# bitlayer-org/tap-stark

Measured on AMD Instinct MI355X. Metric: trace cells/sec (proofs/sec alongside), 2^20x64 BabyBear trace, higher is better.
Workload: dtype u32

## Files before the change

tap-stark_amd/csrc/abi.cpp:

```cpp
#include <stdio.h>
#include <string.h>

#include <algorithm>
#include <atomic>
#include <chrono>
#include <mutex>
#include <thread>
#include <memory>
#include <string>
#include <vector>

#include "abi_types.hpp"
#include "blake3.hpp"
#include "collect.hpp"
#include "derive.hpp"
#include "jit.hpp"
#include "join.hpp"
#include "logup.hpp"
#include "prover_internal.hpp"
#include "scan.hpp"
#include "sort.hpp"

static const ts::AirProgram& ready_prog(const ts_air* air) { return const_cast<ts_air*>(air)->a.ready(); }

// ... 438 lines not shown
    memcpy(buf, s.c_str(), s.size() + 1);
    return TS_OK;
}

ts_status ts_ctx_set_replay(ts_ctx* ctx, int mode) {
    if (!ctx || mode < 0 || mode > 2) return TS_ERR_INVALID;
    return guard(ctx, [&] {
        ctx->ctx.sync();
        if (mode == 1) ctx->ctx.replay_log.clear();
        ctx->ctx.replay_pos = 0;
        ctx->ctx.replay_mode = mode;
    });
}
ts_status ts_ctx_set_kernel_timing(ts_ctx* ctx, int enabled) {
    if (!ctx) return TS_ERR_INVALID;
    return guard(ctx, [&] {
        ctx->ctx.take_kernel_timings();
        ctx->ctx.kernel_timing = enabled != 0;
    });
}
ts_status ts_ctx_take_kernel_timings(ts_ctx* ctx, char* buf, size_t cap) {
    if (!ctx || !buf || cap == 0) return TS_ERR_INVALID;
    return guard(ctx, [&] {
        std::string s;
        for (auto& kv : ctx->ctx.take_kernel_timings()) {
            char tmp[200];
            snprintf(tmp, sizeof tmp, "%s=%llu:%.6f;", kv.first.c_str(),
                     (unsigned long long)kv.second.first, kv.second.second);
            s += tmp;
        }
        TS_REQUIRE(s.size() + 1 <= cap, ts::TS_ERR_BUFFER, "timing buffer too small");
        memcpy(buf, s.c_str(), s.size() + 1);
    });
}

ts_status ts_ctx_graph_stats(ts_ctx* ctx, uint64_t out[4]) {
    if (!ctx || !out) return TS_ERR_INVALID;
    out[0] = out[1] = out[2] = 0;
    out[3] = ctx->ctx.bytes_reserved;
    return TS_OK;
}

ts_status ts_ctx_stat(ts_ctx* ctx, int which, uint64_t* out) {
    if (!ctx || !out) return TS_ERR_INVALID;
    switch (which) {
    case 0: case 1: case 2: case 4: *out = 0; break;
    case 3: *out = ctx->ctx.bytes_reserved; break;
    case 5: *out = ctx->ctx.local_quotient_fallbacks; break;
    case 6: *out = ctx->ctx.pow_hints_accepted; break;
    case 7: *out = ctx->ctx.pow_hints_rejected; break;
    case 8: *out = ctx->ctx.pow_host_grinds; break;
    case 9: *out = ctx->ctx.poison_fills; break;
    case 11: *out = ctx->ctx.live_blocks.size(); break;
    default: return TS_ERR_INVALID;
    }
    return TS_OK;
}

ts_status ts_bench_alu(ts_ctx* ctx, int kind, double* units_per_second) {
    if (!ctx || !units_per_second) return TS_ERR_INVALID;
    return guard(ctx, [&] { *units_per_second = ts::alu_ceiling(ctx->ctx, kind); });
}

ts_status ts_bench_stage(ts_ctx* ctx, int stage, unsigned log_n, uint32_t width, unsigned log_blowup,
                         uint32_t reps, double* ms_per_rep) {
    if (!ctx || !ms_per_rep) return TS_ERR_INVALID;
    return guard(ctx, [&] { *ms_per_rep = ts::bench_stage(ctx->ctx, stage, log_n, width, log_blowup, reps); });
}

ts_status ts_host_alloc(size_t bytes, void** out) {
    if (!out || bytes == 0) return TS_ERR_INVALID;
    *out = nullptr;
    return hipHostMalloc(out, bytes, hipHostMallocDefault) == hipSuccess ? TS_OK : TS_ERR_OOM;
}
void ts_host_free(void* p) {
    if (p) (void)hipHostFree(p);
}

static ts_matrix* new_matrix(ts::DeviceMatrix m) {
    auto h = std::make_unique<ts_matrix>();
    h->m = std::move(m);
    return h.release();
}
static ts_status matrix_from(ts_ctx* ctx, const uint32_t* src, uint64_t height, uint32_t width,
                             hipMemcpyKind kind, ts_matrix** out, bool sync = true) {
    if (!ctx || !out) return TS_ERR_INVALID;
    *out = nullptr;
    return guard(ctx, [&] {
        TS_REQUIRE(src && height >= 1 && width >= 1, ts::TS_ERR_INVALID, "matrix: empty");
        TS_REQUIRE((height & (height - 1)) == 0, ts::TS_ERR_INVALID, "matrix: height must be a power of two");
        TS_REQUIRE(height <= (1ull << 27), ts::TS_ERR_INVALID, "matrix: height > 2^27");
        auto m = std::make_unique<ts_matrix>();
        m->m.buf = ts::DevBuf<uint32_t>(&ctx->ctx, (size_t)height * width);
        m->m.height = height;
        m->m.width = width;
        m->m.layout = ts::DeviceMatrix::ROW_MAJOR;
        TS_HIP(hipMemcpyAsync(m->m.buf.p, src, (size_t)height * width * 4, kind, ctx->ctx.stream));
        if (sync) ctx->ctx.sync();
        *out = m.release();
    });
}
ts_status ts_matrix_upload(ts_ctx* ctx, const uint32_t* host, uint64_t height, uint32_t width,
                           ts_matrix** out) {
    return matrix_from(ctx, host, height, width, hipMemcpyHostToDevice, out);
}
ts_status ts_matrix_upload_async(ts_ctx* ctx, const uint32_t* host_pinned, uint64_t height,
// ... 2012 lines not shown
```

tap-stark_amd/csrc/context.cpp:

```cpp
#include <errno.h>
#include <stdio.h>
#include <time.h>
#include <stdlib.h>
#include "context.hpp"

#include <string.h>

#include "kernels.hpp"

namespace ts {

static bool poison_knob(uint32_t* word) {
    const char* e = getenv("TS_POOL_POISON");
    if (!e || !*e) return false;
    char* end = nullptr;
    errno = 0;
    const unsigned long v = strtoul(e, &end, 0);
    TS_REQUIRE(errno == 0 && end != e && *end == 0 && e[0] != '-' && v <= 0xFFFFFFFFul, TS_ERR_INVALID,
               "TS_POOL_POISON is not a 32-bit word (decimal, 0x hex or 0 octal)");
    *word = (uint32_t)v;
    return true;
}

Context::Context(int dev) : device(dev) {
    pool_debug = getenv("TS_POOL_DEBUG") != nullptr;
    poison_on = poison_knob(&poison_word);
    int count = 0;
    hipError_t e = hipGetDeviceCount(&count);
    if (e != hipSuccess || count == 0)
        throw Error(TS_ERR_HIP, "no HIP device available: the tap-stark HIP path has no CPU fallback");
    TS_REQUIRE(dev >= 0 && dev < count, TS_ERR_INVALID, "device index out of range");
    TS_HIP(hipSetDevice(dev));
    hipDeviceProp_t prop;
    TS_HIP(hipGetDeviceProperties(&prop, dev));
    num_cus = prop.multiProcessorCount;
    max_lds_per_block = prop.sharedMemPerBlock;
    arch_name = prop.gcnArchName;
    arch_name = arch_name.substr(0, arch_name.find(':'));
    TS_HIP(hipStreamCreateWithFlags(&stream, hipStreamNonBlocking));
}

Context::~Context() {
    (void)hipSetDevice(device);
    if (stream) (void)hipStreamSynchronize(stream);
    if (d_twiddle_fwd) (void)hipFree(d_twiddle_fwd);
    if (d_twiddle_inv) (void)hipFree(d_twiddle_inv);
    if (d_plant_fwd) (void)hipFree(d_plant_fwd);
    if (d_plant_inv) (void)hipFree(d_plant_inv);
    for (auto& t : scale_tables) (void)hipFree(t.d);
    for (auto& t : sel_tables)
        if (t.d) (void)hipFree(t.d);
    if (d_ticket) (void)hipFree(d_ticket);
    for (auto& kv : free_blocks) (void)hipFree(kv.second);
    for (auto& kv : live_blocks) (void)hipFree(kv.first);
    if (h_pinned) (void)hipHostFree(h_pinned);
    if (h_mailbox) (void)hipHostFree(h_mailbox);
    if (h_mailbox_big) (void)hipHostFree(h_mailbox_big);
    if (h_arena) (void)hipHostFree(h_arena);
    if (stream) (void)hipStreamDestroy(stream);
}

static size_t round_block(size_t bytes) {
    if (bytes < 512) return 512;
    if (bytes < (1u << 20)) {
        size_t r = 512;
        while (r < bytes) r <<= 1;
        return r;
    }
    const size_t g = 1u << 20;
    return (bytes + g - 1) / g * g;
}

void* Context::alloc(size_t bytes) {
    const size_t sz = round_block(bytes);
    auto it = free_blocks.find(sz);
    void* p = nullptr;
    if (it != free_blocks.end()) {
        p = it->second;
        free_blocks.erase(it);
    } else {
        TS_HIP(hipSetDevice(device));
        if (pool_debug) {
            struct timespec ts_;
            clock_gettime(CLOCK_MONOTONIC, &ts_);
            fprintf(stderr, "[ts pool %p t=%.3f ms] hipMalloc %zu KiB (reserved %zu MiB)\n", (void*)this,
                    ts_.tv_sec * 1e3 + ts_.tv_nsec * 1e-6, sz >> 10, bytes_reserved >> 20);
        }
        hipError_t e = hipMalloc(&p, sz);
        if (e != hipSuccess) {
            release_cache();
            e = hipMalloc(&p, sz);
        }
        if (e != hipSuccess) {
            (void)hipGetLastError();
            throw Error(TS_ERR_OOM, "device allocation failed");
        }
        bytes_reserved += sz;
    }
    live_blocks[p] = sz;
    if (poison_on) poison(p, sz);
    return p;
}

void Context::poison(void* p, size_t bytes) {
// ... 6 lines not shown
void Context::free(void* p) {
    if (!p) return;
    auto it = live_blocks.find(p);
    if (it == live_blocks.end()) return;
    free_blocks.emplace(it->second, p);
    live_blocks.erase(it);
}

void Context::release_cache() {
    if (stream) (void)hipStreamSynchronize(stream);
    for (auto& kv : free_blocks) {
        (void)hipFree(kv.second);
        bytes_reserved -= kv.first;
    }
    free_blocks.clear();
}

uint32_t* Context::ticket() {
    if (!d_ticket) {
        TS_HIP(hipMalloc((void**)&d_ticket, 64 * 17));
        TS_HIP(hipMemsetAsync(d_ticket, 0, 64 * 17, stream));
    }
    return d_ticket;
}

const void* Context::stage(const void* src, size_t bytes) {
    const size_t need = (bytes + 63) & ~(size_t)63;
    if (need > h_arena_bytes / 2) {
        sync();
        if (h_arena) (void)hipHostFree(h_arena);
        h_arena = nullptr;
        size_t sz = 1 << 20;
        while (sz / 2 < need) sz <<= 1;
        TS_HIP(hipHostMalloc((void**)&h_arena, sz, hipHostMallocDefault));
        h_arena_bytes = sz;
        h_arena_off = 0;
    }
    if (h_arena_off + need > h_arena_bytes) {
        sync();
        h_arena_off = 0;
    }
    void* p = h_arena + h_arena_off;
    memcpy(p, src, bytes);
    h_arena_off += need;
    return p;
}

void Context::sync_point(void* host, size_t bytes) {
    if (replay_mode == 2 && replay_pos < replay_log.size() && replay_log[replay_pos].size() == bytes) {
        memcpy(host, replay_log[replay_pos++].data(), bytes);
        return;
    }
    sync();
    if (replay_mode == 1) replay_log.emplace_back((const char*)host, (const char*)host + bytes);
}
void Context::d2h_point(void* host_dst, const void* dev_src, size_t bytes) {
    if (replay_mode == 2 && replay_pos < replay_log.size() && replay_log[replay_pos].size() == bytes) {
        memcpy(host_dst, replay_log[replay_pos++].data(), bytes);
        return;
    }
    if (bytes) TS_HIP(hipMemcpyAsync(host_dst, dev_src, bytes, hipMemcpyDeviceToHost, stream));
    sync();
    if (replay_mode == 1) replay_log.emplace_back((const char*)host_dst, (const char*)host_dst + bytes);
}

uint32_t* Context::mailbox(size_t words) {
    constexpr size_t WORDS = 16384;
    if (words > WORDS / 4) {
        if (words > h_mailbox_big_words) {
            sync();
            if (h_mailbox_big) (void)hipHostFree(h_mailbox_big);
            h_mailbox_big = nullptr;
            h_mailbox_big_words = 0;
            TS_HIP(hipHostMalloc((void**)&h_mailbox_big, words * 4, hipHostMallocDefault));
            h_mailbox_big_words = words;
        }
        return h_mailbox_big;
    }
    if (!h_mailbox) TS_HIP(hipHostMalloc((void**)&h_mailbox, WORDS * 4, hipHostMallocDefault));
    const size_t need = (words + 15) & ~(size_t)15;
    if (mailbox_off + need > WORDS) mailbox_off = 0;
    uint32_t* p = h_mailbox + mailbox_off;
    mailbox_off += need;
    return p;
}

void* Context::pinned(size_t bytes) {
    if (bytes > h_pinned_bytes) {
        if (h_pinned) {
            sync();
            (void)hipHostFree(h_pinned);
        }
        size_t sz = 1 << 16;
        while (sz < bytes) sz <<= 1;
        TS_HIP(hipHostMalloc(&h_pinned, sz, hipHostMallocDefault));
        h_pinned_bytes = sz;
    }
    return h_pinned;
}

std::map<std::string, std::pair<uint64_t, double>> Context::take_kernel_timings() {
    std::map<std::string, std::pair<uint64_t, double>> out;
    sync();
    for (auto& ev : kernel_events) {
        float ms = 0;
        (void)hipEventElapsedTime(&ms, ev.e0, ev.e1);
        auto& slot = out[ev.name];
        slot.first += 1;
        slot.second += ms;
        (void)hipEventDestroy(ev.e0);
        (void)hipEventDestroy(ev.e1);
    }
    kernel_events.clear();
    return out;
}

void Context::ensure_twiddles(unsigned log_size) {
    if (log_size <= twiddle_log && d_twiddle_fwd) return;
    TS_REQUIRE(log_size <= 27, TS_ERR_INVALID, "two-adicity of BabyBear is 27");
    sync();
    if (d_twiddle_fwd) (void)hipFree(d_twiddle_fwd);
    if (d_twiddle_inv) (void)hipFree(d_twiddle_inv);
    d_twiddle_fwd = d_twiddle_inv = nullptr;
    const size_t n = (size_t)1 << log_size;
    TS_HIP(hipMalloc((void**)&d_twiddle_fwd, n * 4));
    TS_HIP(hipMalloc((void**)&d_twiddle_inv, n * 4));
    if (poison_on) {
        poison(d_twiddle_fwd, n * 4);
        poison(d_twiddle_inv, n * 4);
    }
    twiddle_log = log_size;
    launch_build_twiddles(*this, d_twiddle_fwd, d_twiddle_inv, log_size);
}

void Context::ensure_plant_twiddles(unsigned log_size) {
    if (log_size <= plant_log && d_plant_fwd) return;
    TS_REQUIRE(log_size <= 27, TS_ERR_INVALID, "two-adicity of BabyBear is 27");
    sync();
    if (d_plant_fwd) (void)hipFree(d_plant_fwd);
    if (d_plant_inv) (void)hipFree(d_plant_inv);
    d_plant_fwd = d_plant_inv = nullptr;
    const size_t n = (size_t)1 << log_size;
    TS_HIP(hipMalloc((void**)&d_plant_fwd, n * 8));
    TS_HIP(hipMalloc((void**)&d_plant_inv, n * 8));
    if (poison_on) {
        poison(d_plant_fwd, n * 8);
        poison(d_plant_inv, n * 8);
    }
    plant_log = log_size;
    launch_build_plant_twiddles(*this, d_plant_fwd, d_plant_inv, log_size);
}

}
```

tap-stark_amd/csrc/context.hpp:

```cpp
#pragma once
#include <hip/hip_runtime.h>
#include <stdint.h>

#include <map>
#include <stdexcept>
#include <string>
#include <vector>

#include "bb.hpp"

namespace ts {

struct Error : std::runtime_error {
    int code;
    Error(int c, const std::string& m) : std::runtime_error(m), code(c) {}
};

struct FinalPolyNotConstant : Error {
    explicit FinalPolyNotConstant(const std::string& m) : Error(5 , m) {}
};

enum : int {
    TS_OK = 0,
    TS_ERR_INVALID = 1,
    TS_ERR_HIP = 2,
    TS_ERR_OOM = 3,
    TS_ERR_UNSUPPORTED = 4,
    TS_ERR_INVARIANT = 5,
    TS_ERR_BUFFER = 6,
    TS_ERR_COMM = 7,
};

#define TS_HIP(expr)                                                                        \
    do {                                                                                    \
        hipError_t _e = (expr);                                                             \
        if (_e != hipSuccess)                                                               \
            throw ts::Error(ts::TS_ERR_HIP, std::string(#expr) + ": " + hipGetErrorString(_e)); \
    } while (0)

#define TS_REQUIRE(cond, code, msg)                   \
    do {                                              \
        if (!(cond)) throw ts::Error((code), (msg));  \
    } while (0)

struct Context {
    int device = 0;
    hipStream_t stream = nullptr;
    std::string last_error;
    int num_cus = 256;
    size_t max_lds_per_block = 64 * 1024;
    std::string arch_name;

    std::multimap<size_t, void*> free_blocks;
    std::map<void*, size_t> live_blocks;
    size_t bytes_reserved = 0;
    bool pool_debug = false;
    bool poison_on = false;
    uint32_t poison_word = 0;
    uint64_t poison_fills = 0;
    void poison(void* p, size_t bytes);

    uint32_t* d_twiddle_fwd = nullptr;
    uint32_t* d_twiddle_inv = nullptr;
    unsigned twiddle_log = 0;
    uint2* d_plant_fwd = nullptr;
    uint2* d_plant_inv = nullptr;
    unsigned plant_log = 0;

    struct ScaleTable {
        unsigned log_n, log_blowup;
        uint32_t shift;
        uint32_t* d;
        size_t words;
        uint64_t last_use;
    };
    std::vector<ScaleTable> scale_tables;
    uint64_t scale_clock = 0;
    struct SelTable {
        uint32_t* d = nullptr;
        unsigned log_n = ~0u, log_qd = ~0u;
        uint32_t shift = 0;
        uint64_t last_use = 0;
    };
    SelTable sel_tables[2];
    uint64_t sel_clock = 0;

    uint32_t* d_ticket = nullptr;
    uint32_t* ticket();

    unsigned lde_pass_mask = 7;

    uint32_t* h_mailbox = nullptr;
    size_t mailbox_off = 0;
    uint32_t* h_mailbox_big = nullptr;
    size_t h_mailbox_big_words = 0;
    uint32_t* mailbox(size_t words);

    void* h_pinned = nullptr;
    size_t h_pinned_bytes = 0;
    char* h_arena = nullptr;
    size_t h_arena_bytes = 0, h_arena_off = 0;
    const void* stage(const void* src, size_t bytes);

    bool timing = false;
    std::vector<std::pair<std::string, float>> stage_ms;

    struct KernelEvent {
        const char* name;
        hipEvent_t e0, e1;
    };
    bool kernel_timing = false;
    std::vector<KernelEvent> kernel_events;
    std::map<std::string, std::pair<uint64_t, double>> take_kernel_timings();

    uint64_t pow_hints_accepted = 0, pow_hints_rejected = 0, pow_host_grinds = 0;
    uint64_t local_quotient_fallbacks = 0;

    explicit Context(int dev);
    ~Context();
    Context(const Context&) = delete;

    void* alloc(size_t bytes);
    void free(void* p);
    template <class T>
    T* alloc_n(size_t n) { return static_cast<T*>(alloc(n * sizeof(T))); }
    void release_cache();

    int replay_mode = 0;
    size_t replay_pos = 0;
    std::vector<std::vector<char>> replay_log;
    void sync_point(void* host, size_t bytes);
    void d2h_point(void* host_dst, const void* dev_src, size_t bytes);
    void* pinned(size_t bytes);
    void ensure_twiddles(unsigned log_size);
    void ensure_plant_twiddles(unsigned log_size);
    void sync() { TS_HIP(hipStreamSynchronize(stream)); }
};

// ... 77 lines not shown
```

tap-stark_amd/csrc/ntt.hip:

```cpp
#include "kernels.hpp"

namespace ts {

constexpr int SHIFT_LO_BITS = 10;

__device__ __forceinline__ uint32_t twiddle_mont(uint32_t idx) {
    if (idx == 0) return R_MOD_P;
    unsigned logm = 31 - __clz(idx);
    uint32_t i = idx - (1u << logm);
    uint32_t g27 = to_mont(TWO_ADIC_GEN_27);
    uint32_t g = mont_pow(g27, 1ull << (27 - (logm + 1)));
    uint32_t e = bitrev32(i, logm);
    return mont_pow(g, e);
}

__global__ void k_build_twiddles(uint32_t* __restrict__ W, uint32_t* __restrict__ Winv,
                                 unsigned log_size) {
    uint32_t idx = blockIdx.x * blockDim.x + threadIdx.x;
    if (idx >= (1u << log_size)) return;
    const uint32_t w = twiddle_mont(idx);
    W[idx] = w;
    Winv[idx] = mont_inv(w);
}

// ... 7 lines not shown
}

void launch_build_twiddles(Context& ctx, uint32_t* W, uint32_t* Winv, unsigned log_size) {
    uint32_t n = 1u << log_size;
    TS_LAUNCH(ctx, k_build_twiddles, dim3((n + 255) / 256), dim3(256), 0, W, Winv, log_size);
    TS_HIP(hipGetLastError());
}

void launch_build_plant_twiddles(Context& ctx, uint2* WP, uint2* WPinv, unsigned log_size) {
    uint32_t n = 1u << log_size;
    TS_LAUNCH(ctx, k_build_plant_twiddles, dim3((n + 255) / 256), dim3(256), 0, WP, WPinv, log_size);
    TS_HIP(hipGetLastError());
}

__global__ void k_build_shift_tables(uint32_t* __restrict__ lo, uint32_t* __restrict__ hi,
                                     uint32_t n_hi, uint32_t shift_mont, unsigned log_N,
                                     unsigned log_blowup, uint32_t scale_mont) {
    uint32_t beta = blockIdx.y;
    uint32_t j = blockIdx.x * blockDim.x + threadIdx.x;
    uint32_t n_lo = 1u << SHIFT_LO_BITS;
    if (j >= n_lo + n_hi) return;
    uint32_t g27 = to_mont(TWO_ADIC_GEN_27);
    uint32_t gN = mont_pow(g27, 1ull << (27 - log_N));
    uint32_t s = mont_mul(shift_mont, mont_pow(gN, bitrev32(beta, log_blowup)));
    if (j < n_lo) {
        lo[beta * n_lo + j] = mont_mul(mont_pow(s, j), scale_mont);
    } else {
        uint32_t jj = j - n_lo;
        hi[beta * n_hi + jj] = mont_pow(s, (uint64_t)jj << SHIFT_LO_BITS);
    }
}

void launch_build_shift_tables(Context& ctx, uint32_t* lo, uint32_t* hi, uint32_t n_hi,
                               uint32_t n_cosets, uint32_t shift_mont, unsigned log_N,
                               unsigned log_blowup, uint32_t scale_mont) {
    const uint32_t n_lo = 1u << SHIFT_LO_BITS;
    TS_LAUNCH(ctx, k_build_shift_tables, dim3((n_lo + n_hi + 255) / 256, n_cosets), dim3(256), 0, lo,
              hi, n_hi, shift_mont, log_N, log_blowup, scale_mont);
    TS_HIP(hipGetLastError());
}

__global__ void __launch_bounds__(256)
k_build_scale_table(const uint32_t* __restrict__ lo, const uint32_t* __restrict__ hi, uint32_t n_hi,
                    unsigned log_n, uint32_t* __restrict__ T) {
    const uint32_t beta = blockIdx.y;
    const uint64_t k = (uint64_t)blockIdx.x * blockDim.x + threadIdx.x;
    if (k >= (1ull << log_n)) return;
    const uint32_t n_lo = 1u << SHIFT_LO_BITS;
    T[((uint64_t)beta << log_n) + k] =
        mont_mul(lo[beta * n_lo + (k & (n_lo - 1))], hi[(uint64_t)beta * n_hi + (k >> SHIFT_LO_BITS)]);
}

const uint32_t* coset_scale_table(Context& ctx, unsigned log_n, unsigned log_blowup, uint32_t shift) {
    for (auto& t : ctx.scale_tables)
        if (t.log_n == log_n && t.log_blowup == log_blowup && t.shift == shift) {
            t.last_use = ++ctx.scale_clock;
            return t.d;
        }
    const uint32_t n_cosets = 1u << log_blowup;
    const size_t words = (size_t)n_cosets << log_n;
    size_t total = words * 4;
    for (auto& t : ctx.scale_tables) total += t.words * 4;
    while (!ctx.scale_tables.empty() && (ctx.scale_tables.size() >= 8 || total > (2ull << 30))) {
        size_t victim = 0;
        for (size_t i = 1; i < ctx.scale_tables.size(); i++)
            if (ctx.scale_tables[i].last_use < ctx.scale_tables[victim].last_use) victim = i;
        ctx.sync();
        total -= ctx.scale_tables[victim].words * 4;
        (void)hipFree(ctx.scale_tables[victim].d);
        ctx.scale_tables.erase(ctx.scale_tables.begin() + victim);
    }
    uint32_t* d = nullptr;
    TS_HIP(hipMalloc((void**)&d, words * 4));
    if (ctx.poison_on) ctx.poison(d, words * 4);
    const uint64_t n = 1ull << log_n;
    const uint32_t n_lo = 1u << SHIFT_LO_BITS;
    const uint32_t n_hi = log_n > (unsigned)SHIFT_LO_BITS ? 1u << (log_n - SHIFT_LO_BITS) : 1u;
    DevBuf<uint32_t> lo(&ctx, (size_t)n_cosets * n_lo), hi(&ctx, (size_t)n_cosets * n_hi);
    const uint32_t n_inv_mont = to_mont(inv_canon((uint32_t)(n % P)));
    launch_build_shift_tables(ctx, lo.p, hi.p, n_hi, n_cosets, to_mont(shift), log_n + log_blowup, log_blowup,
                              n_inv_mont);
    TS_LAUNCH(ctx, k_build_scale_table, dim3((unsigned)((n + 255) / 256), n_cosets), dim3(256), 0,
              (const uint32_t*)lo.p, (const uint32_t*)hi.p, n_hi, log_n, d);
    TS_HIP(hipGetLastError());
    ctx.scale_tables.push_back(Context::ScaleTable{log_n, log_blowup, shift, d, words, ++ctx.scale_clock});
    return d;
}

template <bool TO_COLUMNS, bool BITREV>
__global__ void __launch_bounds__(256)
k_transpose_tile(const uint32_t* __restrict__ src, uint32_t* __restrict__ dst, uint64_t h, unsigned log_h,
                 uint32_t w, uint64_t col_stride, uint32_t rm_width) {
    __shared__ uint32_t tile[64][65];
    const uint64_t p0 = (uint64_t)blockIdx.x * 64;
    const uint32_t c0 = blockIdx.y * 64;
    const uint32_t tx = threadIdx.x & 63, ty = threadIdx.x >> 6;
    auto row_of = [&](uint64_t p) -> uint64_t { return BITREV ? bitrev32((uint32_t)p, log_h) : p; };
    if (p0 + 64 <= h && c0 + 64 <= w) {
        const uint64_t rm = row_of(p0) * rm_width + c0 + tx;
        const uint64_t rm_step = BITREV ? (uint64_t)rm_width << (log_h - 6) : rm_width;
        const uint64_t cm = (uint64_t)(c0 + ty) * col_stride + p0 + tx;
        auto rm_at = [&](int k) {
            const uint32_t i = ty + 4 * (uint32_t)k;
            return rm + (uint64_t)(BITREV ? __brev(i) >> 26 : i) * rm_step;
        };
        auto cm_at = [&](int k) { return cm + (uint64_t)(4 * k) * col_stride; };
        uint32_t t[16];
#pragma unroll
        for (int k = 0; k < 16; k++) t[k] = src[TO_COLUMNS ? rm_at(k) : cm_at(k)];
#pragma unroll
        for (int k = 0; k < 16; k++) (TO_COLUMNS ? tile[ty + 4 * k][tx] : tile[tx][ty + 4 * k]) = t[k];
        __syncthreads();
#pragma unroll
        for (int k = 0; k < 16; k++) t[k] = TO_COLUMNS ? tile[tx][ty + 4 * k] : tile[ty + 4 * k][tx];
#pragma unroll
        for (int k = 0; k < 16; k++) dst[TO_COLUMNS ? cm_at(k) : rm_at(k)] = t[k];
        return;
    }
    auto rm_ok = [&](uint32_t j) { return p0 + j < h && c0 + tx < w; };
    auto cm_ok = [&](uint32_t j) { return c0 + j < w && p0 + tx < h; };
    auto rm_at = [&](uint32_t j) { return row_of(p0 + j) * rm_width + c0 + tx; };
    auto cm_at = [&](uint32_t j) { return (uint64_t)(c0 + j) * col_stride + p0 + tx; };
#pragma unroll
    for (int k = 0; k < 16; k++) {
        const uint32_t j = ty + 4 * (uint32_t)k;
        if (TO_COLUMNS ? rm_ok(j) : cm_ok(j)) (TO_COLUMNS ? tile[j][tx] : tile[tx][j]) = src[TO_COLUMNS ? rm_at(j) : cm_at(j)];
    }
    __syncthreads();
#pragma unroll
    for (int k = 0; k < 16; k++) {
        const uint32_t j = ty + 4 * (uint32_t)k;
        if (TO_COLUMNS ? cm_ok(j) : rm_ok(j)) dst[TO_COLUMNS ? cm_at(j) : rm_at(j)] = TO_COLUMNS ? tile[tx][j] : tile[j][tx];
    }
}

template <bool TO_COLUMNS, bool BITREV>
static void launch_transpose_tile(Context& ctx, const char* name, const uint32_t* src, uint32_t* dst, uint64_t h,
                                  unsigned log_h, uint32_t w, uint64_t col_stride, uint32_t rm_width) {
    if (w == 0 || h == 0) return;
// ... 28 lines not shown
```

tap-stark_amd/csrc/ntt_lde.hip:

```cpp
#include <stdlib.h>

#include <optional>
#include <type_traits>

#include "ntt_rounds.hpp"

namespace ts {

template <int LM, bool SKIP_R16 = false, class TW = uint32_t>
__global__ void __launch_bounds__(chunk_threads(LM))
k_intt_contig(uint32_t* __restrict__ data, uint64_t col_stride, unsigned log_n,
              const TW* __restrict__ Winv, uint32_t* __restrict__ data2, uint32_t gw) {
    __shared__ uint32_t s[padded(1 << LM)];
    const uint32_t c = blockIdx.x;
    uint32_t* col = blockIdx.y < gw ? data + (uint64_t)blockIdx.y * col_stride
                                    : data2 + (uint64_t)(blockIdx.y - gw) * col_stride;
    uint32_t* g = col + ((uint64_t)c << LM);
    chunk_load<LM>(s, g);
    chunk_rounds<LM, true, SKIP_R16>(s, log_n - LM, c, Winv);
    chunk_store<LM, false>(s, g);
}

__global__ void __launch_bounds__(256)
k_transpose_bitrev_r16(const uint32_t* __restrict__ src, uint32_t* __restrict__ dst, unsigned log_n,
// ... 330 lines not shown
        TS_LAUNCH_NAMED(ctx, "k_lde_mid<1>", TS_MID_K(1, TILE_ELEMS, LOG_M, false), grid1, b, 0, TS_MID_ARGS);
    else if (p.mid == NttMid::FIXED256 && p.LM == 13)
        TS_LAUNCH_NAMED(ctx, "(k_lde_mid<1, 8192, 512, 13>)", TS_MID_K(1, 8192, 13, false), grid1, b, 0, TS_MID_ARGS);
    else if (p.mid == NttMid::FIXED256)
        TS_LAUNCH_NAMED(ctx, "(k_lde_mid<1, 8192, 512, 14>)", TS_MID_K(1, 8192, 14, false), grid1, b, 0, TS_MID_ARGS);
    else
        TS_LAUNCH_NAMED(ctx, "k_lde_mid<0>", TS_MID_K(0, TILE_ELEMS, LOG_M, false), grid, b, 0, TS_MID_ARGS);
#undef TS_MID_ARGS
#undef TS_MID_K
}

void launch_contig_forward(Context& ctx, const NttPlan& p, uint32_t* data, uint64_t col_stride, uint32_t ncols,
                           uint32_t n_blocks, uint32_t gw, uint32_t own_a, uint32_t own_b) {
    const TwTables W = twiddles_fwd(ctx);
    with_chunk_log(p.LM, [&](auto lm) {
        constexpr int LM = decltype(lm)::value;
        using TW = typename ContigForm<LM>::Fwd;
        constexpr int CPW = LM == 14 ? 4 : 1;
        if (own_a != LDE_NO_OWN)
            TS_LAUNCH_NAMED(ctx, FWD_NAME[LM - 12], (k_lde_fwd_contig_own<LM, CPW, TW>),
                            dim3(p.chunks / CPW, ncols, n_blocks - 1), dim3(chunk_threads(LM)), 0, data, col_stride,
                            p.log_n, W, gw, own_a, own_b);
        else
            TS_LAUNCH_NAMED(ctx, FWD_NAME[LM - 12], (k_lde_fwd_contig<LM, CPW, TW>), dim3(p.chunks / CPW, ncols, n_blocks),
                            dim3(chunk_threads(LM)), 0, data, col_stride, p.log_n, W);
    });
}

int lde_own_coset_used(unsigned log_n, unsigned log_blowup, uint32_t shift) {
    if (const char* e = getenv("TS_LDE_OWN_COSET"); e && *e && atoi(e) == 0) return -1;
    if (log_blowup == 0 || log_n + log_blowup > 27 || ntt_plan(log_n).mid == NttMid::TILE16384) return -1;
    return lde_own_coset(log_n, log_blowup, shift);
}

void coset_lde(Context& ctx, uint32_t* evals, uint64_t in_col_stride, uint32_t ncols, unsigned log_n,
               unsigned log_blowup, uint32_t shift, uint32_t* out, uint64_t out_col_stride,
               uint32_t beta0, uint32_t n_beta, bool first_round_done, uint32_t* evals2, uint32_t shift2,
               uint32_t gw, bool stage_timers) {
    if (ncols == 0) return;
    TS_REQUIRE(evals2 == nullptr || (gw >= 1 && gw < ncols && shift2 != 0), TS_ERR_INVALID,
               "coset_lde: second matrix needs its first column and its shift");
    if (evals2 == nullptr) gw = 0xffffffffu;
    TS_REQUIRE(log_n + log_blowup <= 27, TS_ERR_INVALID, "coset_lde: log_n + log_blowup > 27");
    const NttPlan p = ntt_plan(log_n);
    ntt_require_shape(p, ncols, in_col_stride, out_col_stride, true);
    TS_REQUIRE(!first_round_done || p.fused_first_round, TS_ERR_INVARIANT,
               "coset_lde: no contiguous inverse pass at this size");
    ctx.ensure_twiddles(log_n == 0 ? 1 : log_n);
    ctx.ensure_plant_twiddles(log_n == 0 ? 1 : log_n);

    const uint32_t n_cosets = 1u << log_blowup;
    if (n_beta == 0) n_beta = n_cosets - beta0;
    TS_REQUIRE(beta0 < n_cosets && n_beta <= n_cosets - beta0, TS_ERR_INVALID, "coset_lde: coset range");
    const uint32_t* scale = coset_scale_table(ctx, log_n, log_blowup, shift);
    const uint32_t* scale2 = evals2 ? coset_scale_table(ctx, log_n, log_blowup, shift2) : nullptr;

    uint32_t own_a = LDE_NO_OWN, own_b = LDE_NO_OWN;
    if (beta0 == 0 && n_beta == n_cosets && !first_round_done && ctx.lde_pass_mask == 7u) {
        const int a = lde_own_coset_used(log_n, log_blowup, shift);
        const int b = evals2 ? lde_own_coset_used(log_n, log_blowup, shift2) : a;
        if (a >= 0 && b >= 0) {
            own_a = (uint32_t)a;
            own_b = (uint32_t)b;
            const uint64_t n = 1ull << log_n;
            if (p.two_pass)
                TS_LAUNCH_NAMED(ctx, "k_lde_own_copy", k_lde_own_copy<true>, dim3((unsigned)(n >> 12), ncols), dim3(256), 0,
                                (const uint32_t*)evals, in_col_stride, out, out_col_stride, log_n,
                                (const uint32_t*)evals2, gw, own_a, own_b);
            else
                TS_LAUNCH_NAMED(ctx, "k_lde_own_copy", k_lde_own_copy<false>, dim3((unsigned)((n + 255) / 256), ncols),
                                dim3(256), 0, (const uint32_t*)evals, in_col_stride, out, out_col_stride, log_n,
                                (const uint32_t*)evals2, gw, own_a, own_b);
        }
    }

    if (!p.two_pass) {
        launch_lde_mid(ctx, p, evals, in_col_stride, out, out_col_stride, ncols, beta0, n_beta, scale, evals2, scale2,
                       gw, own_a, own_b);
    } else {
        if (ctx.lde_pass_mask & 1u) {
            std::optional<StageTimer> t;
            if (stage_timers) t.emplace(&ctx, "lde: inverse NTT, contiguous stages");
            launch_contig_inverse(ctx, p, evals, in_col_stride, ncols, first_round_done, evals2, gw);
        }
        std::optional<StageTimer> t_rest;
        if (stage_timers) t_rest.emplace(&ctx, "lde: strided pass + forward NTT of the owned cosets");
        if (ctx.lde_pass_mask & 2u)
            launch_lde_mid(ctx, p, evals, in_col_stride, out, out_col_stride, ncols, beta0, n_beta, scale, evals2,
                           scale2, gw, own_a, own_b);
        if (ctx.lde_pass_mask & 4u) launch_contig_forward(ctx, p, out, out_col_stride, ncols, n_beta, gw, own_a, own_b);
    }
    TS_HIP(hipGetLastError());
}

}
```

tap-stark_amd/csrc/quotient.hip:

```cpp
#include <stdlib.h>

#include <algorithm>

#include "air.hpp"
#include "kernels.hpp"

namespace ts {

constexpr int SEL_BATCH = 8;

struct SelConsts {
    uint32_t zh_mont[MAX_QUOTIENT_CHUNKS];
};

__global__ void __launch_bounds__(256)
k_selectors(unsigned L, unsigned log_qd, const uint32_t* __restrict__ W, uint32_t gen_mont,
            uint32_t gn_inv_mont, SelConsts sc, uint32_t* __restrict__ is_first,
            uint32_t* __restrict__ is_last, uint32_t* __restrict__ is_transition) {
    const uint64_t total = 1ull << L;
    const uint64_t r0 = ((uint64_t)blockIdx.x * blockDim.x + threadIdx.x) * SEL_BATCH;
    if (r0 >= total) return;
    const unsigned log_n = L - log_qd;
    uint32_t d[2 * SEL_BATCH];
    uint32_t pre[2 * SEL_BATCH];
    uint32_t run = R_MOD_P;
    const int cnt = (total - r0) < (uint64_t)SEL_BATCH ? (int)(total - r0) : SEL_BATCH;
#pragma unroll
    for (int k = 0; k < SEL_BATCH; k++) {
        if (k < cnt) {
            uint64_t r = r0 + k;
            uint32_t w = L == 0 ? R_MOD_P : W[(total >> 1) + (r >> 1)];
            if (r & 1) w = neg(w);
            uint32_t x = mont_mul(gen_mont, w);
            d[2 * k] = sub(x, R_MOD_P);
            d[2 * k + 1] = sub(x, gn_inv_mont);
        } else {
            d[2 * k] = d[2 * k + 1] = R_MOD_P;
        }
        pre[2 * k] = run;
        run = mont_mul(run, d[2 * k]);
        pre[2 * k + 1] = run;
        run = mont_mul(run, d[2 * k + 1]);
    }
    uint32_t inv = mont_inv(run);
#pragma unroll
    for (int k = SEL_BATCH - 1; k >= 0; k--) {
        uint32_t inv_last = mont_mul(inv, pre[2 * k + 1]);
        inv = mont_mul(inv, d[2 * k + 1]);
        uint32_t inv_first = mont_mul(inv, pre[2 * k]);
        inv = mont_mul(inv, d[2 * k]);
        if (k < cnt) {
            uint64_t r = r0 + k;
            uint32_t c = bitrev32((uint32_t)(r >> log_n), log_qd);
            uint32_t zh = sc.zh_mont[c];
            is_first[r] = mont_mul(zh, inv_first);
            is_last[r] = mont_mul(zh, inv_last);
            is_transition[r] = d[2 * k + 1];
        }
    }
}

static void coset_vanishing(uint32_t shift, unsigned log_n, unsigned log_qd, uint32_t zh[MAX_QUOTIENT_CHUNKS]) {
    TS_REQUIRE((1u << log_qd) <= (unsigned)MAX_QUOTIENT_CHUNKS, TS_ERR_UNSUPPORTED, "quotient degree > 64 not supported");
    const uint32_t s_pow_n = pow_canon(shift, 1ull << log_n);
    const uint32_t gqd = two_adic_generator(log_qd);
    for (uint32_t c = 0; c < (1u << log_qd); c++) zh[c] = sub(mul(s_pow_n, pow_canon(gqd, c)), 1);
}

static void launch_selectors(Context& ctx, unsigned log_n, unsigned log_qd, uint32_t* is_first,
                             uint32_t* is_last, uint32_t* is_transition, uint32_t shift) {
    const unsigned L = log_n + log_qd;
    ctx.ensure_twiddles(L == 0 ? 1 : L);
    SelConsts sc;
    coset_vanishing(shift, log_n, log_qd, sc.zh_mont);
    for (uint32_t c = 0; c < (1u << log_qd); c++) sc.zh_mont[c] = to_mont(sc.zh_mont[c]);
    const uint32_t gn_inv = inv_canon(two_adic_generator(log_n));
    const uint64_t threads = (((uint64_t)1 << L) + SEL_BATCH - 1) / SEL_BATCH;
    TS_LAUNCH(ctx, k_selectors, dim3((unsigned)((threads + 255) / 256)), dim3(256), 0, L, log_qd, ctx.d_twiddle_fwd, to_mont(shift), to_mont(gn_inv), sc, is_first,
                       is_last, is_transition);
    TS_HIP(hipGetLastError());
}

const uint32_t* selector_table(Context& ctx, unsigned log_n, unsigned log_qd, uint32_t shift) {
    Context::SelTable* st = nullptr;
    for (auto& t : ctx.sel_tables)
        if (t.d && t.log_n == log_n && t.log_qd == log_qd && t.shift == shift) st = &t;
    if (!st) {
        st = ctx.sel_tables[0].last_use <= ctx.sel_tables[1].last_use ? &ctx.sel_tables[0] : &ctx.sel_tables[1];
        if (st->d) {
            ctx.sync();
            (void)hipFree(st->d);
            *st = Context::SelTable{};
        }
        const uint64_t qn = 1ull << (log_n + log_qd);
        TS_HIP(hipMalloc((void**)&st->d, 3 * qn * sizeof(uint32_t)));
        if (ctx.poison_on) ctx.poison(st->d, 3 * qn * sizeof(uint32_t));
        launch_selectors(ctx, log_n, log_qd, st->d, st->d + qn, st->d + 2 * qn, shift);
        st->log_n = log_n;
        st->log_qd = log_qd;
        st->shift = shift;
    }
    st->last_use = ++ctx.sel_clock;
    return st->d;
}

struct QuotConsts {
    uint32_t inv_zh_canonical[MAX_QUOTIENT_CHUNKS];
};

struct RegFilePlan {
    int nthreads;
    bool global;
    size_t lds_bytes;
    unsigned grid;
    uint32_t n_tiles;
    size_t scratch_words;
};

static uint64_t env_u64(const char* name, uint64_t dflt) {
    const char* e = getenv(name);
    return e && *e ? (uint64_t)atoi(e) : dflt;
}

static RegFilePlan plan_reg_file(Context& ctx, uint32_t n_regs, uint64_t rows) {
    RegFilePlan pl;
    pl.nthreads = 256;
    while (pl.nthreads > 64 && (size_t)n_regs * pl.nthreads * 4 > 48 * 1024) pl.nthreads >>= 1;
    pl.lds_bytes = (size_t)n_regs * pl.nthreads * 4;
    const size_t lds_max_regs = env_u64("TS_INTERP_LDS_MAX_REGS", 48);
    const unsigned waves_per_cu = (unsigned)env_u64("TS_INTERP_WAVES_PER_CU", 16);
    pl.global = n_regs > lds_max_regs || pl.lds_bytes > ctx.max_lds_per_block || getenv("TS_INTERP_GLOBAL_REGS") != nullptr;
    if (pl.global) pl.nthreads = 64;
    pl.n_tiles = (uint32_t)((rows + pl.nthreads - 1) / pl.nthreads);
    if (pl.global) {
        pl.lds_bytes = 0;
        uint64_t grid = std::min<uint64_t>(pl.n_tiles, (uint64_t)ctx.num_cus * waves_per_cu);
        const uint64_t slab_mb = env_u64("TS_INTERP_SLAB_MB", 4096);
        const uint64_t cap = (slab_mb << 18) / ((uint64_t)n_regs * 64);
        grid = std::max<uint64_t>(1, std::min(grid, cap));
        pl.grid = (unsigned)grid;
    } else {
        pl.grid = pl.n_tiles;
    }
    pl.scratch_words = pl.global ? (size_t)pl.grid * n_regs * 64 : 0;
    return pl;
}

template <int NTHREADS, bool GLOBAL_REGS>
__device__ __forceinline__ uint32_t* lane_regs(uint32_t* reg_slabs, uint32_t n_regs) {
    extern __shared__ uint32_t lds_regs[];
    return GLOBAL_REGS ? reg_slabs + (size_t)blockIdx.x * n_regs * NTHREADS + threadIdx.x : lds_regs + threadIdx.x;
}

template <int NTHREADS, class Row>
__device__ __forceinline__ void run_program(const uint32_t* code, uint32_t n_instr,
                                            const uint32_t* consts_mont, uint32_t* my, Row& row) {
// ... 329 lines not shown
```

Baseline: 26.58 billion.

## Share twiddle, scale and selector tables across contexts on the same device

Moves twiddle, plant-twiddle, coset scale and selector tables into a per-device registry shared by all contexts through reference-counted handles with LRU eviction, so several contexts or provers on one GPU reuse tables instead of each rebuilding them. The selector cache grows from 2 to 16 entries when shared. Builds now synchronize the stream, and refs to evicted tables are dropped at sync points. This adds mutex and ref-count bookkeeping and can raise device memory residency.

```diff
diff --git a/tap-stark_amd/csrc/abi.cpp b/tap-stark_amd/csrc/abi.cpp
--- a/tap-stark_amd/csrc/abi.cpp
+++ b/tap-stark_amd/csrc/abi.cpp
@@ -514,6 +514,8 @@
     case 8: *out = ctx->ctx.pow_host_grinds; break;
     case 9: *out = ctx->ctx.poison_fills; break;
     case 11: *out = ctx->ctx.live_blocks.size(); break;
+    case 12: *out = ctx->ctx.table_bytes(); break;
+    case 13: *out = ctx->ctx.tables_built; break;
     default: return TS_ERR_INVALID;
     }
     return TS_OK;
diff --git a/tap-stark_amd/csrc/context.cpp b/tap-stark_amd/csrc/context.cpp
--- a/tap-stark_amd/csrc/context.cpp
+++ b/tap-stark_amd/csrc/context.cpp
@@ -38,18 +38,16 @@
     arch_name = prop.gcnArchName;
     arch_name = arch_name.substr(0, arch_name.find(':'));
     TS_HIP(hipStreamCreateWithFlags(&stream, hipStreamNonBlocking));
+    tables = device_tables(dev, poison_on || !shared_tables_knob());
 }
 
 Context::~Context() {
     (void)hipSetDevice(device);
     if (stream) (void)hipStreamSynchronize(stream);
-    if (d_twiddle_fwd) (void)hipFree(d_twiddle_fwd);
-    if (d_twiddle_inv) (void)hipFree(d_twiddle_inv);
-    if (d_plant_fwd) (void)hipFree(d_plant_fwd);
-    if (d_plant_inv) (void)hipFree(d_plant_inv);
-    for (auto& t : scale_tables) (void)hipFree(t.d);
-    for (auto& t : sel_tables)
-        if (t.d) (void)hipFree(t.d);
+    table_refs.held.clear();
+    twiddle_ref.reset();
+    plant_ref.reset();
+    tables.reset();
     if (d_ticket) (void)hipFree(d_ticket);
     for (auto& kv : free_blocks) (void)hipFree(kv.second);
     for (auto& kv : live_blocks) (void)hipFree(kv.first);
@@ -162,6 +160,7 @@
         return;
     }
     sync();
+    table_refs.drop_evicted();
     if (replay_mode == 1) replay_log.emplace_back((const char*)host, (const char*)host + bytes);
 }
 void Context::d2h_point(void* host_dst, const void* dev_src, size_t bytes) {
@@ -171,6 +170,7 @@
     }
     if (bytes) TS_HIP(hipMemcpyAsync(host_dst, dev_src, bytes, hipMemcpyDeviceToHost, stream));
     sync();
+    table_refs.drop_evicted();
     if (replay_mode == 1) replay_log.emplace_back((const char*)host_dst, (const char*)host_dst + bytes);
 }
 
@@ -226,39 +226,41 @@
 }
 
 void Context::ensure_twiddles(unsigned log_size) {
-    if (log_size <= twiddle_log && d_twiddle_fwd) return;
+    if (d_twiddle_fwd && log_size <= twiddle_log && twiddle_log == tables->twiddle_log(TAB_TWIDDLE)) return;
     TS_REQUIRE(log_size <= 27, TS_ERR_INVALID, "two-adicity of BabyBear is 27");
-    sync();
-    if (d_twiddle_fwd) (void)hipFree(d_twiddle_fwd);
-    if (d_twiddle_inv) (void)hipFree(d_twiddle_inv);
-    d_twiddle_fwd = d_twiddle_inv = nullptr;
     const size_t n = (size_t)1 << log_size;
-    TS_HIP(hipMalloc((void**)&d_twiddle_fwd, n * 4));
-    TS_HIP(hipMalloc((void**)&d_twiddle_inv, n * 4));
-    if (poison_on) {
-        poison(d_twiddle_fwd, n * 4);
-        poison(d_twiddle_inv, n * 4);
-    }
-    twiddle_log = log_size;
-    launch_build_twiddles(*this, d_twiddle_fwd, d_twiddle_inv, log_size);
+    bool built = false;
+    twiddle_ref = tables->twiddles(TAB_TWIDDLE, log_size, n * 4, [&](void* fwd, void* inv) {
+        if (poison_on) {
+            poison(fwd, n * 4);
+            poison(inv, n * 4);
+        }
+        launch_build_twiddles(*this, (uint32_t*)fwd, (uint32_t*)inv, log_size);
+        sync();
+    }, &built);
+    tables_built += built;
+    d_twiddle_fwd = (uint32_t*)twiddle_ref->d[0];
+    d_twiddle_inv = (uint32_t*)twiddle_ref->d[1];
+    twiddle_log = twiddle_ref->key.a;
 }
 
 void Context::ensure_plant_twiddles(unsigned log_size) {
-    if (log_size <= plant_log && d_plant_fwd) return;
+    if (d_plant_fwd && log_size <= plant_log && plant_log == tables->twiddle_log(TAB_PLANT)) return;
     TS_REQUIRE(log_size <= 27, TS_ERR_INVALID, "two-adicity of BabyBear is 27");
-    sync();
-    if (d_plant_fwd) (void)hipFree(d_plant_fwd);
-    if (d_plant_inv) (void)hipFree(d_plant_inv);
-    d_plant_fwd = d_plant_inv = nullptr;
     const size_t n = (size_t)1 << log_size;
-    TS_HIP(hipMalloc((void**)&d_plant_fwd, n * 8));
-    TS_HIP(hipMalloc((void**)&d_plant_inv, n * 8));
-    if (poison_on) {
-        poison(d_plant_fwd, n * 8);
-        poison(d_plant_inv, n * 8);
-    }
-    plant_log = log_size;
-    launch_build_plant_twiddles(*this, d_plant_fwd, d_plant_inv, log_size);
-}
-
-}
+    bool built = false;
+    plant_ref = tables->twiddles(TAB_PLANT, log_size, n * 8, [&](void* fwd, void* inv) {
+        if (poison_on) {
+            poison(fwd, n * 8);
+            poison(inv, n * 8);
+        }
+        launch_build_plant_twiddles(*this, (uint2*)fwd, (uint2*)inv, log_size);
+        sync();
+    }, &built);
+    tables_built += built;
+    d_plant_fwd = (uint2*)plant_ref->d[0];
+    d_plant_inv = (uint2*)plant_ref->d[1];
+    plant_log = plant_ref->key.a;
+}
+
+}
diff --git a/tap-stark_amd/csrc/context.hpp b/tap-stark_amd/csrc/context.hpp
--- a/tap-stark_amd/csrc/context.hpp
+++ b/tap-stark_amd/csrc/context.hpp
@@ -8,6 +8,7 @@
 #include <vector>
 
 #include "bb.hpp"
+#include "device_tables.hpp"
 
 namespace ts {
 
@@ -60,30 +61,38 @@
     uint64_t poison_fills = 0;
     void poison(void* p, size_t bytes);
 
+    std::shared_ptr<DeviceTables> tables;
     uint32_t* d_twiddle_fwd = nullptr;
     uint32_t* d_twiddle_inv = nullptr;
     unsigned twiddle_log = 0;
+    TableRef twiddle_ref;
     uint2* d_plant_fwd = nullptr;
     uint2* d_plant_inv = nullptr;
     unsigned plant_log = 0;
-
-    struct ScaleTable {
-        unsigned log_n, log_blowup;
-        uint32_t shift;
-        uint32_t* d;
-        size_t words;
-        uint64_t last_use;
-    };
-    std::vector<ScaleTable> scale_tables;
-    uint64_t scale_clock = 0;
-    struct SelTable {
-        uint32_t* d = nullptr;
-        unsigned log_n = ~0u, log_qd = ~0u;
-        uint32_t shift = 0;
-        uint64_t last_use = 0;
-    };
-    SelTable sel_tables[2];
-    uint64_t sel_clock = 0;
+    TableRef plant_ref;
+
+    TableRefs<HipTableAlloc> table_refs;
+    uint64_t tables_built = 0;
+    template <class Build>
+    const uint32_t* keyed_table(const TableKey& key, size_t bytes, Build&& build) {
+        if (TableRef r = table_refs.find(key)) {
+            tables->touch(*r);
+            return static_cast<const uint32_t*>(r->d[0]);
+        }
+        bool built = false;
+        TableRef r = tables->keyed(key, bytes, build, &built);
+        tables_built += built;
+        table_refs.hold(r);
+        return static_cast<const uint32_t*>(r->d[0]);
+    }
+    void trim_table_refs() {
+        if (!table_refs.any_evicted()) return;
+        sync();
+        table_refs.drop_evicted();
+    }
+    size_t table_bytes() const {
+        return table_refs.bytes() + (twiddle_ref ? twiddle_ref->bytes : 0) + (plant_ref ? plant_ref->bytes : 0);
+    }
 
     uint32_t* d_ticket = nullptr;
     uint32_t* ticket();
diff --git a/tap-stark_amd/csrc/device_tables.cpp b/tap-stark_amd/csrc/device_tables.cpp
--- /dev/null
+++ b/tap-stark_amd/csrc/device_tables.cpp
@@ -0,0 +1,48 @@
+#include "device_tables.hpp"
+
+#include <stdlib.h>
+
+#include <map>
+
+#include "context.hpp"
+
+namespace ts {
+
+void* HipTableAlloc::alloc(size_t bytes) {
+    void* p = nullptr;
+    TS_HIP(hipSetDevice(device));
+    if (hipMalloc(&p, bytes) != hipSuccess) {
+        (void)hipGetLastError();
+        throw Error(TS_ERR_OOM, "device allocation of a table failed");
+    }
+    return p;
+}
+
+void HipTableAlloc::free(void* p) {
+    (void)hipSetDevice(device);
+    (void)hipFree(p);
+}
+
+bool shared_tables_knob() {
+    const char* e = getenv("TS_SHARED_TABLES");
+    return !e || !*e || atoi(e) != 0;
+}
+
+static std::shared_ptr<DeviceTables> make_tables(int device, bool private_set) {
+    const DeviceTables::Limit scale{8, (size_t)2 << 30}, selector{private_set ? 2u : 16u, (size_t)2 << 30};
+    return std::make_shared<DeviceTables>(HipTableAlloc{device}, scale, selector);
+}
+
+std::shared_ptr<DeviceTables> device_tables(int device, bool private_set) {
+    if (private_set) return make_tables(device, true);
+    static std::mutex* mu = new std::mutex;
+    static auto* by_device = new std::map<int, std::weak_ptr<DeviceTables>>;
+    std::lock_guard<std::mutex> lock(*mu);
+    auto& slot = (*by_device)[device];
+    if (auto t = slot.lock()) return t;
+    auto t = make_tables(device, false);
+    slot = t;
+    return t;
+}
+
+}
diff --git a/tap-stark_amd/csrc/device_tables.hpp b/tap-stark_amd/csrc/device_tables.hpp
--- /dev/null
+++ b/tap-stark_amd/csrc/device_tables.hpp
@@ -0,0 +1,176 @@
+#pragma once
+#include <stddef.h>
+#include <stdint.h>
+
+#include <atomic>
+#include <memory>
+#include <mutex>
+#include <vector>
+
+namespace ts {
+
+enum TableFamily : unsigned { TAB_TWIDDLE = 0, TAB_PLANT = 1, TAB_SCALE = 2, TAB_SELECTOR = 3, TAB_FAMILIES = 4 };
+
+struct TableKey {
+    unsigned family = 0, a = 0, b = 0;
+    uint32_t shift = 0;
+    bool operator==(const TableKey& o) const { return family == o.family && a == o.a && b == o.b && shift == o.shift; }
+};
+
+template <class Alloc>
+struct DeviceTable {
+    TableKey key;
+    void* d[2] = {nullptr, nullptr};
+    size_t bytes = 0;
+    Alloc alloc{};
+    mutable std::atomic<uint64_t> last_use{0};
+    std::atomic<bool> evicted{false};
+
+    DeviceTable() = default;
+    DeviceTable(const DeviceTable&) = delete;
+    ~DeviceTable() {
+        for (void* p : d)
+            if (p) alloc.free(p);
+    }
+};
+
+template <class Alloc>
+class TableRegistry {
+public:
+    using Table = DeviceTable<Alloc>;
+    using Ref = std::shared_ptr<const Table>;
+
+    struct Limit {
+        size_t max_tables, max_bytes;
+    };
+
+    TableRegistry(Alloc a, Limit scale, Limit selector) : alloc_(std::move(a)), limit_{{0, 0}, {0, 0}, scale, selector} {}
+    TableRegistry(const TableRegistry&) = delete;
+
+    unsigned twiddle_log(unsigned family) const { return twiddle_log_[family].load(std::memory_order_acquire); }
+
+    template <class Build>
+    Ref twiddles(unsigned family, unsigned log_size, size_t buffer_bytes, Build&& build, bool* built) {
+        std::lock_guard<std::mutex> lock(mu_);
+        *built = false;
+        if (current_[family] && current_[family]->key.a >= log_size) return current_[family];
+        auto t = make(TableKey{family, log_size, 0, 0}, buffer_bytes, 2);
+        build(t->d[0], t->d[1]);
+        if (current_[family]) superseded_.push_back(current_[family]);
+        current_[family] = t;
+        twiddle_log_[family].store(log_size, std::memory_order_release);
+        *built = true;
+        return t;
+    }
+
+    template <class Build>
+    Ref keyed(const TableKey& key, size_t buffer_bytes, Build&& build, bool* built) {
+        std::lock_guard<std::mutex> lock(mu_);
+        *built = false;
+        auto& fam = keyed_[key.family];
+        for (auto& t : fam)
+            if (t->key == key) {
+                touch(*t);
+                return t;
+            }
+        const Limit lim = limit_[key.family];
+        size_t total = buffer_bytes;
+        for (auto& t : fam) total += t->bytes;
+        while (!fam.empty() && (fam.size() >= lim.max_tables || total > lim.max_bytes)) {
+            size_t victim = 0;
+            for (size_t i = 1; i < fam.size(); i++)
+                if (fam[i]->last_use.load(std::memory_order_relaxed) < fam[victim]->last_use.load(std::memory_order_relaxed))
+                    victim = i;
+            total -= fam[victim]->bytes;
+            fam[victim]->evicted.store(true, std::memory_order_release);
+            fam.erase(fam.begin() + victim);
+        }
+        auto t = make(key, buffer_bytes, 1);
+        build(t->d[0]);
+        touch(*t);
+        fam.push_back(t);
+        *built = true;
+        return t;
+    }
+
+    void touch(const Table& t) { t.last_use.store(clock_.fetch_add(1, std::memory_order_relaxed) + 1, std::memory_order_relaxed); }
+
+    size_t published(unsigned family) {
+        std::lock_guard<std::mutex> lock(mu_);
+        return family < TAB_SCALE ? (current_[family] ? 1 : 0) : keyed_[family].size();
+    }
+    size_t superseded() {
+        std::lock_guard<std::mutex> lock(mu_);
+        return superseded_.size();
+    }
+
+private:
+    std::shared_ptr<Table> make(const TableKey& key, size_t buffer_bytes, int buffers) {
+        auto t = std::make_shared<Table>();
+        t->key = key;
+        t->alloc = alloc_;
+        for (int i = 0; i < buffers; i++) {
+            t->d[i] = alloc_.alloc(buffer_bytes);
+            t->bytes += buffer_bytes;
+        }
+        return t;
+    }
+
+    Alloc alloc_;
+    std::mutex mu_;
+    Limit limit_[TAB_FAMILIES];
+    std::shared_ptr<Table> current_[2];
+    std::atomic<unsigned> twiddle_log_[2] = {{0}, {0}};
+    std::vector<std::shared_ptr<Table>> superseded_;
+    std::vector<std::shared_ptr<Table>> keyed_[TAB_FAMILIES];
+    std::atomic<uint64_t> clock_{0};
+};
+
+template <class Alloc>
+struct TableRefs {
+    using Ref = typename TableRegistry<Alloc>::Ref;
+    std::vector<Ref> held;
+
+    Ref find(const TableKey& key) const {
+        for (auto& r : held)
+            if (r->key == key && !r->evicted.load(std::memory_order_acquire)) return r;
+        return nullptr;
+    }
+    void hold(const Ref& r) {
+        for (auto& h : held)
+            if (h == r) return;
+        held.push_back(r);
+    }
+    bool any_evicted() const {
+        for (auto& r : held)
+            if (r->evicted.load(std::memory_order_acquire)) return true;
+        return false;
+    }
+    void drop_evicted() {
+        size_t k = 0;
+        for (size_t i = 0; i < held.size(); i++)
+            if (!held[i]->evicted.load(std::memory_order_acquire)) {
+                if (k != i) held[k] = std::move(held[i]);
+                k++;
+            }
+        held.resize(k);
+    }
+    size_t bytes() const {
+        size_t b = 0;
+        for (auto& r : held) b += r->bytes;
+        return b;
+    }
+};
+
+struct HipTableAlloc {
+    int device;
+    void* alloc(size_t bytes);
+    void free(void* p);
+};
+using DeviceTables = TableRegistry<HipTableAlloc>;
+using TableRef = DeviceTables::Ref;
+
+std::shared_ptr<DeviceTables> device_tables(int device, bool private_set);
+bool shared_tables_knob();
+
+}
diff --git a/tap-stark_amd/csrc/ntt.hip b/tap-stark_amd/csrc/ntt.hip
--- a/tap-stark_amd/csrc/ntt.hip
+++ b/tap-stark_amd/csrc/ntt.hip
@@ -83,39 +83,23 @@
 }
 
 const uint32_t* coset_scale_table(Context& ctx, unsigned log_n, unsigned log_blowup, uint32_t shift) {
-    for (auto& t : ctx.scale_tables)
-        if (t.log_n == log_n && t.log_blowup == log_blowup && t.shift == shift) {
-            t.last_use = ++ctx.scale_clock;
-            return t.d;
-        }
     const uint32_t n_cosets = 1u << log_blowup;
     const size_t words = (size_t)n_cosets << log_n;
-    size_t total = words * 4;
-    for (auto& t : ctx.scale_tables) total += t.words * 4;
-    while (!ctx.scale_tables.empty() && (ctx.scale_tables.size() >= 8 || total > (2ull << 30))) {
-        size_t victim = 0;
-        for (size_t i = 1; i < ctx.scale_tables.size(); i++)
-            if (ctx.scale_tables[i].last_use < ctx.scale_tables[victim].last_use) victim = i;
+    return ctx.keyed_table(TableKey{TAB_SCALE, log_n, log_blowup, shift}, words * 4, [&](void* table) {
+        uint32_t* d = static_cast<uint32_t*>(table);
+        if (ctx.poison_on) ctx.poison(d, words * 4);
+        const uint64_t n = 1ull << log_n;
+        const uint32_t n_lo = 1u << SHIFT_LO_BITS;
+        const uint32_t n_hi = log_n > (unsigned)SHIFT_LO_BITS ? 1u << (log_n - SHIFT_LO_BITS) : 1u;
+        DevBuf<uint32_t> lo(&ctx, (size_t)n_cosets * n_lo), hi(&ctx, (size_t)n_cosets * n_hi);
+        const uint32_t n_inv_mont = to_mont(inv_canon((uint32_t)(n % P)));
+        launch_build_shift_tables(ctx, lo.p, hi.p, n_hi, n_cosets, to_mont(shift), log_n + log_blowup, log_blowup,
+                                  n_inv_mont);
+        TS_LAUNCH(ctx, k_build_scale_table, dim3((unsigned)((n + 255) / 256), n_cosets), dim3(256), 0,
+                  (const uint32_t*)lo.p, (const uint32_t*)hi.p, n_hi, log_n, d);
+        TS_HIP(hipGetLastError());
         ctx.sync();
-        total -= ctx.scale_tables[victim].words * 4;
-        (void)hipFree(ctx.scale_tables[victim].d);
-        ctx.scale_tables.erase(ctx.scale_tables.begin() + victim);
-    }
-    uint32_t* d = nullptr;
-    TS_HIP(hipMalloc((void**)&d, words * 4));
-    if (ctx.poison_on) ctx.poison(d, words * 4);
-    const uint64_t n = 1ull << log_n;
-    const uint32_t n_lo = 1u << SHIFT_LO_BITS;
-    const uint32_t n_hi = log_n > (unsigned)SHIFT_LO_BITS ? 1u << (log_n - SHIFT_LO_BITS) : 1u;
-    DevBuf<uint32_t> lo(&ctx, (size_t)n_cosets * n_lo), hi(&ctx, (size_t)n_cosets * n_hi);
-    const uint32_t n_inv_mont = to_mont(inv_canon((uint32_t)(n % P)));
-    launch_build_shift_tables(ctx, lo.p, hi.p, n_hi, n_cosets, to_mont(shift), log_n + log_blowup, log_blowup,
-                              n_inv_mont);
-    TS_LAUNCH(ctx, k_build_scale_table, dim3((unsigned)((n + 255) / 256), n_cosets), dim3(256), 0,
-              (const uint32_t*)lo.p, (const uint32_t*)hi.p, n_hi, log_n, d);
-    TS_HIP(hipGetLastError());
-    ctx.scale_tables.push_back(Context::ScaleTable{log_n, log_blowup, shift, d, words, ++ctx.scale_clock});
-    return d;
+    });
 }
 
 template <bool TO_COLUMNS, bool BITREV>
diff --git a/tap-stark_amd/csrc/ntt_lde.hip b/tap-stark_amd/csrc/ntt_lde.hip
--- a/tap-stark_amd/csrc/ntt_lde.hip
+++ b/tap-stark_amd/csrc/ntt_lde.hip
@@ -406,6 +406,7 @@
     const uint32_t n_cosets = 1u << log_blowup;
     if (n_beta == 0) n_beta = n_cosets - beta0;
     TS_REQUIRE(beta0 < n_cosets && n_beta <= n_cosets - beta0, TS_ERR_INVALID, "coset_lde: coset range");
+    ctx.trim_table_refs();
     const uint32_t* scale = coset_scale_table(ctx, log_n, log_blowup, shift);
     const uint32_t* scale2 = evals2 ? coset_scale_table(ctx, log_n, log_blowup, shift2) : nullptr;
 
diff --git a/tap-stark_amd/csrc/quotient.hip b/tap-stark_amd/csrc/quotient.hip
--- a/tap-stark_amd/csrc/quotient.hip
+++ b/tap-stark_amd/csrc/quotient.hip
@@ -70,7 +70,6 @@
 static void launch_selectors(Context& ctx, unsigned log_n, unsigned log_qd, uint32_t* is_first,
                              uint32_t* is_last, uint32_t* is_transition, uint32_t shift) {
     const unsigned L = log_n + log_qd;
-    ctx.ensure_twiddles(L == 0 ? 1 : L);
     SelConsts sc;
     coset_vanishing(shift, log_n, log_qd, sc.zh_mont);
     for (uint32_t c = 0; c < (1u << log_qd); c++) sc.zh_mont[c] = to_mont(sc.zh_mont[c]);
@@ -82,26 +81,16 @@
 }
 
 const uint32_t* selector_table(Context& ctx, unsigned log_n, unsigned log_qd, uint32_t shift) {
-    Context::SelTable* st = nullptr;
-    for (auto& t : ctx.sel_tables)
-        if (t.d && t.log_n == log_n && t.log_qd == log_qd && t.shift == shift) st = &t;
-    if (!st) {
-        st = ctx.sel_tables[0].last_use <= ctx.sel_tables[1].last_use ? &ctx.sel_tables[0] : &ctx.sel_tables[1];
-        if (st->d) {
-            ctx.sync();
-            (void)hipFree(st->d);
-            *st = Context::SelTable{};
-        }
-        const uint64_t qn = 1ull << (log_n + log_qd);
-        TS_HIP(hipMalloc((void**)&st->d, 3 * qn * sizeof(uint32_t)));
-        if (ctx.poison_on) ctx.poison(st->d, 3 * qn * sizeof(uint32_t));
-        launch_selectors(ctx, log_n, log_qd, st->d, st->d + qn, st->d + 2 * qn, shift);
-        st->log_n = log_n;
-        st->log_qd = log_qd;
-        st->shift = shift;
-    }
-    st->last_use = ++ctx.sel_clock;
-    return st->d;
+    const uint64_t qn = 1ull << (log_n + log_qd);
+    const unsigned L = log_n + log_qd;
+    ctx.trim_table_refs();
+    ctx.ensure_twiddles(L == 0 ? 1 : L);
+    return ctx.keyed_table(TableKey{TAB_SELECTOR, log_n, log_qd, shift}, 3 * qn * sizeof(uint32_t), [&](void* table) {
+        uint32_t* d = static_cast<uint32_t*>(table);
+        if (ctx.poison_on) ctx.poison(d, 3 * qn * sizeof(uint32_t));
+        launch_selectors(ctx, log_n, log_qd, d, d + qn, d + 2 * qn, shift);
+        ctx.sync();
+    });
 }
 
 struct QuotConsts {
```

New measurement: 26.62 billion (median of 3 runs). About the same (+0.2%).
